# Jittor/PointCloudLib

Measured on AMD Instinct MI355X. Metric: point-clouds/sec fwd+bwd, PointNet++ SSG B=32 N=1024, higher is better.
Workload: dtype f32; 1 GPU; PointNet++ SSG cls train step (fwd+bwd+SGD), B=32/GPU, N=1024 xyz+normal, gauss_ball clouds (BASELINE configs[1]); global_batch=32, n_points=1024, parallelism=dp1, launch=eager, grad_overlap=False, cpu_affinity=numa node 1 (gpu0), 128 cpus, world_size=1, sync_bn=False, entry_points=per-stack (pcl_mlp_stack_*_f32)

## Files before the change

include/pcl_hip.h:

```cpp
#ifndef PCL_HIP_H
#define PCL_HIP_H

#include <stddef.h>
#include <stdint.h>

#ifdef __cplusplus
extern "C" {
#endif

#define PCL_OK 0
#define PCL_EINVAL (-1)
#define PCL_EHIP (-2)
#define PCL_ENOSUP (-3)
#define PCL_EWS (-4)

int pcl_version(void);
void pcl_time_tagged_launch(void* start_event, void* stop_event, const char* tag);
void pcl_time_next_launch(void* start_event, void* stop_event);
const char* pcl_last_launch_kernel(void);
const char* pcl_last_error(void);

int pcl_optimal_block(int batch_size);

void pcl_set_fps_tuning(int threads_per_cloud, int issue_priority);
// ... 48 lines not shown
                         int S, int D, float* out, void* stream);
int pcl_three_interp_bwd_f32(const float* gout, const int32_t* idx3, const float* w3, int B, int N,
                             int S, int D, float* gpoints2, void* stream);

int pcl_density_f32(const float* xyz, int B, int N, float bandwidth, float* density_out, void* stream);

int pcl_group_linear_stat_rows(int B, int m);
int pcl_group_linear_f32(const float* xyz, const float* new_xyz, const float* Uf, const float* Wx, const float* feat_small,
                         const float* Wf_small, int CF, int ldw, const int32_t* idx, const int32_t* cnt, const int32_t* group_off,
                         int B, int N, int m, int ns, int C1, float* Y, int32_t* row_meta, int32_t* row_src,
                         float* row_loc , float* row_feat ,
                         double* stats_ws, void* stream);
int pcl_group_linear_bwd_f32(const float* row_loc, const float* row_feat, int CF, const float* dU, const float* Y,
                             const float* a, const float* k1, const float* k2, const float* mu, const int32_t* row_src,
                             const int32_t* n_rows_dev , int B, int N, int C1, float* dUf,
                             float* dWx_part, float* dWf_part, float* dW0, int ldw, int off, void* stream);
int pcl_group_rows_transpose_supported(int N, int m, int ns);
int pcl_group_rows_transpose_i32(const int32_t* row_src, const int32_t* group_off, int B, int N, int m, int ns, int32_t* in_off,
                                 int32_t* in_rows, void* stream);
int pcl_group_linear_bwd_gather_supported(int C1);
void pcl_set_pointconv_paths(int bwd_w_rows);
void pcl_set_scatter_form(int gather);
int pcl_group_linear_bwd_gather_f32(const float* row_loc, const float* dU, const float* Y, const float* a, const float* k1,
                                    const float* k2, const float* mu, const int32_t* in_off, const int32_t* in_rows, int B, int N,
                                    int C1, float* dUf, float* dWx_part, float* dW0, int ldw, void* stream);
int pcl_group_linear_bwd_regen_supported(int C1, int CF);
int pcl_group_linear_bwd_regen_f32(const float* row_loc, const float* row_feat, const float* Wx, const float* Wf_small, int CF, int ldw,
                                   const float* dU, const float* a, const float* k1, const float* k2, const float* mu,
                                   const int32_t* n_rows_dev , int C1, float* dWx_part, float* dWf_part, float* dW0,
                                   int ld0, int off, void* stream);
int pcl_group_linear_bwd_gather_regen_f32(const float* row_loc, const float* dU, const float* Uf, const float* Wx, int ldw, const float* a,
                                          const float* k1, const float* k2, const float* mu, const int32_t* in_off, const int32_t* in_rows,
                                          int B, int N, int C1, float* dUf, float* dWx_part, float* dW0, int ld0, void* stream);

int pcl_head_layer_fwd_f32(const float* X, const float* W, const float* bias, const float* gamma, const float* beta,
                           float* running_mean, float* running_var, int R, int K, int N, int bn_mode, float eps, float momentum,
                           float slope, float* Ypre, float* OUT, float* mean_out, float* invstd_out, void* workspace,
                           size_t workspace_bytes, void* stream);
size_t pcl_head_layer_fwd_workspace_bytes(int R, int K, int N);
int pcl_head_layer_bwd_f32(const float* X, const float* W, const float* dOUT, const float* OUT, const float* Ypre,
                           const float* gamma, const float* mean, const float* invstd, int R, int K, int N, int bn_mode,
                           float slope, float* dY_ws, float* dW, float* dbias, float* dgamma, float* dbeta, float* dX,
                           void* stream);

#define PCL_HEAD_MAX_LAYERS 4
typedef struct pcl_head_layer_t {
    const float* W;
    const float* bias;
    const float* gamma;
    const float* beta;
    float* running_mean;
    float* running_var;
    float* dW;
    float* dbias;
    float* dgamma;
    float* dbeta;
    int32_t K, N, bn_mode;
    float eps, momentum, slope, drop_p;
    int32_t pad_;
} pcl_head_layer_t;
typedef struct pcl_fc_head_t {
    int32_t struct_bytes;
    int32_t n_layers;
    int32_t R;
    int32_t pad_;
    uint64_t seed;
// ... 44 lines not shown
                       const float* in_shift, float in_slope, int P, int Cin, int Cout, float* Y,
                       double* stats_ws, void* stream);
int pcl_linear_fwd_gmax_f32(const float* X, const float* W, const float* bias, const float* in_scale,
                            const float* in_shift, float in_slope, int P, int Cin, int Cout, int ns, float* Y,
                            double* stats_ws, float* gmax, float* gmin, int32_t* gamax, int32_t* gamin, void* stream);
int pcl_group_minmax_finalize_f32(const float* gmax, const float* gmin, const int32_t* gamax, const int32_t* gamin,
                                  const float* scale, const float* shift, float slope, int G, int C, float* out,
                                  int32_t* arg, float* ymax, void* stream);
int pcl_group_minmax_finalize2_f32(const float* gmax, const float* gmin, const int32_t* gamax, const int32_t* gamin,
                                   const float* scale, const float* shift, float slope, int G, int C, float* out,
                                   int32_t* arg, float* ymax, float* out2, int out2_ld, void* stream);
int pcl_group_minmax_finalize_t_f32(const float* gmax, const float* gmin, const int32_t* gamax, const int32_t* gamin,
                                    const float* scale, const float* shift, float slope, int B, int N, int C, float* out,
                                    int32_t* arg, float* ymax, float* out2, int out2_ld, float* out_t, void* stream);
int pcl_bn_finalize_f32(const double* stats_ws, int stat_rows, const float* gamma, const float* beta, int P,
                        int C, float eps, float momentum, float* scale, float* shift, float* mean_out,
                        float* invstd_out, float* running_mean, float* running_var, void* stream);
int pcl_bn_act_max_mean_f32(const float* Y, const float* scale, const float* shift, float slope, int G, int ns, int C, int ldo,
                            float* out_max, float* out_mean, int32_t* arg, void* stream);
int pcl_bn_act_max_mean_bwd_f32(const float* gmax, const float* gmean, int ldg, const int32_t* arg, const float* Y, const float* scale,
                                const float* shift, float slope, int G, int ns, int C, float* du, double* stats_ws,
                                int* stat_rows_out, void* stream);
int pcl_bn_act_max_f32(const float* Y, const float* scale, const float* shift, float slope, int G, int ns,
                       int C, float* out, int32_t* arg, float* ymax, void* stream);
int pcl_bn_act_f32(const float* Y, const float* scale, const float* shift, float slope, int P, int C,
                   float* out, void* stream);
int pcl_bn_act_bwd_f32(const float* gz, const float* Y, const float* scale, const float* shift, float slope,
                       int P, int C, float* du, double* stats_ws, int* stat_rows_out, void* stream);
int pcl_bn_rows_stats_f32(const float* x, const float* g, int P, int C, double* stats_ws, int* stat_rows_out, void* stream);
int pcl_bn_rows_bwd_apply_f32(const float* g, const float* x, const float* a, const float* k1, const float* k2, const float* mean,
                              int P, int C, float* dx, void* stream);
int pcl_maxgrad_prep_f32(const float* gout, const float* out, const float* ymax, float slope, int G, int C,
                         float* gz, double* stats_ws, int* stat_rows_out, void* stream);
int pcl_bn_bwd_consts_f32(const double* stats_ws, int stat_rows, const float* gamma, const float* mean,
                          const float* invstd, int P, int C, float* dgamma, float* dbeta, float* a_out,
                          float* k1, float* k2, float* dbias_zero, void* stream);
int pcl_linear_bwd_dx_f32(const float* dU, const float* Y, const float* a, const float* k1, const float* k2, const float* mu,
                          const int32_t* arg, const float* gz, int ns, const float* W, int P, int Cout,
                          int Cin, const float* Yprev, const float* prev_scale, const float* prev_shift,
                          float prev_slope, float* dUprev, double* stats_ws, void* stream);
void pcl_set_fb_max_blocks(int n);
void pcl_set_fb_two_images(int on);
int pcl_get_fb_two_images(void);
int pcl_sgd_momentum_f32(const uint64_t* params, const uint64_t* grads, const uint64_t* bufs, const int64_t* numel, int n_tensors, double lr,
                         double momentum, double weight_decay, double dampening, void* stream);
void pcl_set_kernel_paths(int fwd_resident, int narrow_stacks, int fused_backward);
void pcl_set_stack_overlap(int side_dw, int max_rows);
int pcl_get_stack_overlap(void);
int pcl_bn_bwd_dy_supported(int P, int C);
int pcl_bn_bwd_dy_f32(const double* stats_ws, int stat_rows, const float* gamma, const float* mean, const float* invstd, int P_bn, int C,
                      float* dgamma, float* dbeta, float* a_out, float* k1, float* k2, float* dbias_zero, const float* dU, const float* Y,
                      const int32_t* arg, const float* gz, int ns, int P, float* dy, void* stream);
size_t pcl_linear_bwd_dw_plain_workspace_bytes(int P, int Cout, int Cin);
int pcl_linear_bwd_dw_plain_f32(const float* dy, const float* Xprev, const float* prev_scale, const float* prev_shift, float prev_slope, int P,
                                int Cout, int Cin, float* dW, void* workspace, size_t workspace_bytes, int dw_ld, void* stream);
int pcl_mlp_fewrow_layer(int P, int Cout, int Cin, int first_layer);
void pcl_set_fewrow_backward(int on);
int pcl_get_fewrow_backward(void);
void pcl_set_dw_tuning(int gx);
int pcl_linear_bwd_pair_supported(int P, int Cout, int Cin, int first_col);
int pcl_linear_bwd_pair_f32(const float* dU, const float* Y, const float* a, const float* k1, const float* k2, const float* mean,
                            const int32_t* arg, const float* gz, int ns, const float* W, const float* Xprev,
                            const float* prev_scale, const float* prev_shift, float prev_slope, int masked, int P, int Cout, int Cin,
                            float* dUprev, double* stats_ws, int first_col, void* workspace, size_t workspace_bytes, void* stream);
int pcl_linear_bwd_pair_finish_f32(const void* workspace, size_t workspace_bytes, int P, int Cout, int Cin, float* dW, int dw_ld,
                                   const double* stats_ws, int stat_rows, const float* gamma_prev, const float* mean_prev,
                                   const float* invstd_prev, int P_bn, float* dgamma_prev, float* dbeta_prev,
                                   float* a_prev, float* k1_prev, float* k2_prev, float* dbias_zero_prev, void* stream);
void pcl_set_bwd_pair(int on);
int pcl_get_bwd_pair(void);
void pcl_set_matrix_form(int form);
int pcl_get_matrix_form(void);
int pcl_linear_bwd_fused_supported(int Cout, int Cin);
int pcl_linear_bwd_fused_stat_rows(int P, int Cin);
size_t pcl_linear_bwd_fused_workspace_bytes(int P, int Cout, int Cin);
int pcl_linear_bwd_fused_rows_f32(const float* dU, const float* Y, const float* a, const float* k1, const float* k2, const float* mu,
                                  const int32_t* arg, const float* gz, int ns, const float* W, int P, int Cout, int Cin,
                                  const float* Yprev, const float* prev_scale, const float* prev_shift, float prev_slope,
                                  float* dUprev, double* stats_ws, void* workspace, size_t workspace_bytes,
                                  const int32_t* row_meta, const int32_t* n_rows_dev, void* stream);
int pcl_linear_bwd_fused_finish_f32(const void* workspace, size_t workspace_bytes, int P, int Cout, int Cin, float* dW,
                                    const double* stats_ws, const float* gamma_prev, const float* mean_prev,
                                    const float* invstd_prev, int P_bn, float* dgamma_prev, float* dbeta_prev, float* a_prev,
                                    float* k1_prev, float* k2_prev, float* dbias_zero_prev, void* stream);
size_t pcl_linear_bwd_dw_workspace_bytes(int P, int Cout, int Cin);
int pcl_linear_bwd_dw_f32(const float* dU, const float* Y, const float* a, const float* k1, const float* k2, const float* mu,
                          const int32_t* arg, const float* gz, int ns, const float* Xprev,
                          const float* prev_scale, const float* prev_shift, float prev_slope, int P, int Cout,
                          int Cin, float* dW, void* workspace, size_t workspace_bytes, void* stream);

#define PCL_STACK_MAX_LAYERS 8
typedef struct pcl_stack_layer_t {
    const float* W;
    const float* bias;
    const float* gamma;
    const float* beta;
    float* running_mean;
    float* running_var;
    float* dW;
    float* dbias;
    float* dgamma;
// ... 176 lines not shown
```

pointcloudlib_amd/csrc/common.h:

```cpp
#pragma once
#include <hip/hip_runtime.h>
#include <hip/hip_ext.h>
#include <stdint.h>
#include <stdio.h>
#include <stdarg.h>
#include <stdlib.h>
#include "../../include/pcl_hip.h"

namespace pcl {

void set_error(const char* fmt, ...);

inline int fail(int code, const char* fmt, ...) {
    char buf[256];
    va_list ap;
    va_start(ap, fmt);
    vsnprintf(buf, sizeof buf, fmt, ap);
    va_end(ap);
    set_error("%s", buf);
    return code;
}

inline int check_launch(const char* what) {
    hipError_t e = hipGetLastError();
// ... 60 lines not shown
}

#define PCL_WAVE 64

__device__ __forceinline__ float sq_dist3(float ax, float ay, float az, float bx, float by, float bz) {
    const float dx = __fsub_rn(ax, bx), dy = __fsub_rn(ay, by), dz = __fsub_rn(az, bz);
    return __fadd_rn(__fadd_rn(__fmul_rn(dx, dx), __fmul_rn(dy, dy)), __fmul_rn(dz, dz));
}

template <int CTRL>
__device__ __forceinline__ unsigned dpp_u32(unsigned v, unsigned old) {
    return (unsigned)__builtin_amdgcn_update_dpp((int)old, (int)v, CTRL, 0xf, 0xf, false);
}

__device__ __forceinline__ unsigned wave_max_u32(unsigned v) {
    v = max(v, dpp_u32<0xB1>(v, v));
    v = max(v, dpp_u32<0x4E>(v, v));
    v = max(v, dpp_u32<0x141>(v, v));
    v = max(v, dpp_u32<0x140>(v, v));
    const unsigned a = __builtin_amdgcn_readlane(v, 0), b = __builtin_amdgcn_readlane(v, 16);
    const unsigned c = __builtin_amdgcn_readlane(v, 32), d = __builtin_amdgcn_readlane(v, 48);
    return max(max(a, b), max(c, d));
}
__device__ __forceinline__ unsigned wave_min_u32(unsigned v) {
    v = min(v, dpp_u32<0xB1>(v, v));
    v = min(v, dpp_u32<0x4E>(v, v));
    v = min(v, dpp_u32<0x141>(v, v));
    v = min(v, dpp_u32<0x140>(v, v));
    const unsigned a = __builtin_amdgcn_readlane(v, 0), b = __builtin_amdgcn_readlane(v, 16);
    const unsigned c = __builtin_amdgcn_readlane(v, 32), d = __builtin_amdgcn_readlane(v, 48);
    return min(min(a, b), min(c, d));
}

__device__ __forceinline__ int lane_id() { return (int)__builtin_amdgcn_mbcnt_hi(~0u, __builtin_amdgcn_mbcnt_lo(~0u, 0u)); }

__device__ __forceinline__ int mbcnt(unsigned long long mask) {
    return (int)__builtin_amdgcn_mbcnt_hi((unsigned)(mask >> 32), __builtin_amdgcn_mbcnt_lo((unsigned)mask, 0u));
}

}
```

pointcloudlib_amd/csrc/compact.hip:

```cpp
#include "common.h"

namespace pcl {

struct GoffMulti { const int32_t* cnt[4]; int32_t* goff[4]; };
__device__ __forceinline__ void group_offsets_body(const int32_t* __restrict__ cnt, int G, int32_t* __restrict__ goff);
__global__ __launch_bounds__(1024) void group_offsets_kernel(const int32_t* __restrict__ cnt, int G, int32_t* __restrict__ goff) {
    group_offsets_body(cnt, G, goff);
}
__global__ __launch_bounds__(1024) void group_offsets_multi_kernel(const GoffMulti a, int G) {
    group_offsets_body(a.cnt[blockIdx.x], G, a.goff[blockIdx.x]);
}
__device__ __forceinline__ void group_offsets_body(const int32_t* __restrict__ cnt, int G, int32_t* __restrict__ goff) {
    __shared__ int part[1024];
    const int t = threadIdx.x;
    const int per = (G + 1023) / 1024;
    const int lo = min(t * per, G), hi = min(lo + per, G);
    int s = 0;
    for (int g = lo; g < hi; ++g) s += max(cnt[g], 1);
    part[t] = s;
    __syncthreads();
    for (int off = 1; off < 1024; off <<= 1) {
        const int v = t >= off ? part[t - off] : 0;
        __syncthreads();
        part[t] += v;
        __syncthreads();
    }
    int run = part[t] - s;
    for (int g = lo; g < hi; ++g) { goff[g] = run; run += max(cnt[g], 1); }
    if (t == 1023) goff[G] = part[1023];
}

__global__ __launch_bounds__(256) void group_compact_kernel(const float* __restrict__ xyz, const float* __restrict__ new_xyz,
                                                            const float* __restrict__ feat, const int32_t* __restrict__ idx,
                                                            const int32_t* __restrict__ cnt, const int32_t* __restrict__ goff,
                                                            int G, int N, int m, int ns, int C, int use_xyz, int S,
                                                            float* __restrict__ rows, int2* __restrict__ rmeta,
                                                            int32_t* __restrict__ rsrc) {
    const int g = blockIdx.x, wave = threadIdx.x >> 6, lane = threadIdx.x & 63;
    const int D = (use_xyz ? 3 : 0) + C, off3 = use_xyz ? 3 : 0;
    const int c = max(cnt[g], 1), base = goff[g];
    const int b = g / m;
    const int32_t* I = idx + (size_t)g * ns;
    const int chunk = (ns + 3) >> 2;
    const int s_lo = wave * chunk, s_hi = min(s_lo + chunk, c);
    if (s_lo >= s_hi) return;
    float* o = rows + (size_t)base * S;
    const float* fb = feat ? feat + (size_t)b * N * C : nullptr;
    if (C >= 32) {
        float q[3] = {0.f, 0.f, 0.f};
        if (use_xyz && lane < 3) q[0] = new_xyz[(size_t)g * 3 + lane];
        for (int s = s_lo; s < s_hi; s += 4) {
            int k[4];
#pragma unroll
            for (int j = 0; j < 4; ++j) k[j] = I[min(s + j, s_hi - 1)];
            for (int c0 = 0; c0 < C; c0 += 128) {
                float v[4][2];
#pragma unroll
                for (int j = 0; j < 4; ++j)
#pragma unroll
                    for (int h = 0; h < 2; ++h) {
                        const int ch = min(c0 + h * 64 + lane, C - 1);
                        v[j][h] = fb[(size_t)k[j] * C + ch];
// ... 698 lines not shown
    __syncthreads();
    int run = inc - s;
    for (int w = 0; w < wave; ++w) run += wtot[w];
    for (int i = i0; i < i1; ++i) {
        const int t = off[i];
        off[i] = run;
        int pos = run;
        for (int w = 0; w < RT_W; ++w) { const int c = cnt[w * N + i]; cnt[w * N + i] = pos; pos += c; }
        run += t;
    }
    if (tid == 0) off[N] = re - rb;
    __syncthreads();
    for (int g = g0; g < g1; ++g) {
        const int q0 = group_off[g_first + g], q1 = group_off[g_first + g + 1];
        for (int r = q0 + lane; r < q1; r += 64) lst[atomicAdd(&mycnt[rsrc[r] - pbase], 1)] = r;
        __builtin_amdgcn_fence(__ATOMIC_SEQ_CST, "wavefront");
        __builtin_amdgcn_wave_barrier();
    }
    __syncthreads();
    for (int pl = tid; pl < N; pl += RT_T) in_off[pbase + pl] = rb + off[pl];
    if (b == B - 1 && tid == 0) in_off[pbase + N] = re;
    for (int i = tid; i < re - rb; i += RT_T) in_rows[rb + i] = lst[i];
}

__global__ __launch_bounds__(256) void group_linear_dw_kernel(const float* __restrict__ px, const float* __restrict__ pf, int rows,
                                                              int C1, int CF, int off, int ld, float* __restrict__ dW0) {
    const int nx = px ? C1 * 3 : 0, nf = pf ? C1 * CF : 0;
    const int e = blockIdx.x * 4 + (threadIdx.x >> 6), lane = threadIdx.x & 63;
    if (e >= nx + nf) return;
    const bool isx = e < nx;
    const float* src = isx ? px + e : pf + (e - nx);
    const int n = isx ? nx : nf;
    float s = 0.f;
    for (int r = lane; r < rows; r += 64) s += src[(size_t)r * n];
#pragma unroll
    for (int o = 32; o > 0; o >>= 1) s += __shfl_xor(s, o);
    if (lane == 0) {
        if (isx) dW0[(size_t)(e / 3) * ld + e % 3] = s;
        else dW0[(size_t)((e - nx) / CF) * ld + off + (e - nx) % CF] = s;
    }
}

}
using namespace pcl;

extern "C" int pcl_group_offsets_i32(const int32_t* cnt, int G, int32_t* group_off, void* stream) {
    PCL_REQUIRE(cnt && group_off && G >= 1, "pcl_group_offsets_i32: bad arguments");
    hipLaunchKernelGGL(group_offsets_kernel, dim3(1), dim3(1024), 0, as_stream(stream), cnt, G, group_off);
    return check_launch("pcl_group_offsets_i32");
}

extern "C" int pcl_group_offsets_multi_i32(int n, const int32_t* const* cnt, int G, int32_t* const* group_off, void* stream) {
    PCL_REQUIRE(cnt && group_off && G >= 1 && n >= 1 && n <= 4, "pcl_group_offsets_multi_i32: bad arguments (n = %d: 1..4)", n);
    GoffMulti a = {};
    for (int i = 0; i < n; ++i) {
        PCL_REQUIRE(cnt[i] && group_off[i], "pcl_group_offsets_multi_i32: null array %d", i);
        a.cnt[i] = cnt[i]; a.goff[i] = group_off[i];
    }
    hipLaunchKernelGGL(group_offsets_multi_kernel, dim3(n), dim3(1024), 0, as_stream(stream), a, G);
    return check_launch("pcl_group_offsets_multi_i32");
}

extern "C" int pcl_group_compact_f32(const float* xyz, const float* new_xyz, const float* feat, const int32_t* idx,
                                     const int32_t* cnt, const int32_t* group_off, int B, int N, int m, int ns, int C,
                                     int use_xyz, int row_stride, float* rows, int32_t* row_meta, int32_t* row_src,
                                     void* stream) {
    PCL_REQUIRE(idx && cnt && rows && row_meta && row_src && group_off, "pcl_group_compact_f32: null pointer");
// ... 106 lines not shown
    return group_linear_bwd_impl(row_loc, row_feat, CF, dU, Y, a, k1, k2, mu, row_src, n_rows_dev, B, N, C1, dUf, dWx_part, dWf_part, dW0, ldw,
                                 off, stream, false);
}
int pcl::group_linear_bwd_impl(const float* row_loc, const float* row_feat, int CF, const float* dU, const float* Y, const float* a,
                               const float* k1, const float* k2, const float* mu, const int32_t* row_src, const int32_t* n_rows_dev, int B,
                               int N, int C1, float* dUf, float* dWx_part, float* dWf_part, float* dW0, int ldw, int off, void* stream,
                               bool duf_is_zero) {
    PCL_REQUIRE(row_loc && dU && Y && a && k1 && k2 && mu && row_src && n_rows_dev, "pcl_group_linear_bwd_f32: null pointer");
    PCL_REQUIRE(dUf || dWx_part || dWf_part, "pcl_group_linear_bwd_f32: nothing to compute");
    PCL_REQUIRE(!dWf_part || (row_feat && CF >= 1 && CF <= GL_CF), "pcl_group_linear_bwd_f32: dWf needs row_feat, CF=%d", CF);
    PCL_REQUIRE(B >= 1 && N >= 1 && C1 >= 1 && C1 <= 64 * GL_MAXH, "pcl_group_linear_bwd_f32: bad sizes");
    PCL_REQUIRE(!dW0 || ((dWx_part || dWf_part) && ldw >= (dWx_part ? 3 : 0) && off >= 0 && ldw >= off + (dWf_part ? CF : 0)),
                "pcl_group_linear_bwd_f32: dW0 needs the partial buffers and ldw=%d >= off=%d + CF", ldw, off);
    hipStream_t st = as_stream(stream);
    if (dUf && !duf_is_zero) {
        hipError_t e = hipMemsetAsync(dUf, 0, sizeof(float) * (size_t)B * N * C1, st);
        if (e != hipSuccess) return fail(PCL_EHIP, "pcl_group_linear_bwd_f32: memset: %s", hipGetErrorString(e));
    }
    const float4* rl = reinterpret_cast<const float4*>(row_loc);
    const float4* rf = reinterpret_cast<const float4*>(row_feat);
    const dim3 grid(GL_BLOCKS), block(256);
    if (!dUf && al16(Y, dU) && (C1 == 64 || C1 == 128 || C1 == 256)) {
        if (C1 == 64) hipLaunchKernelGGL(group_linear_bwd_v4_kernel<16>, grid, block, 0, st, rl, rf, CF, dU, Y, a, k1, k2, mu, row_src, n_rows_dev, dUf, dWx_part, dWf_part);
        else if (C1 == 128) hipLaunchKernelGGL(group_linear_bwd_v4_kernel<32>, grid, block, 0, st, rl, rf, CF, dU, Y, a, k1, k2, mu, row_src, n_rows_dev, dUf, dWx_part, dWf_part);
        else hipLaunchKernelGGL(group_linear_bwd_v4_kernel<64>, grid, block, 0, st, rl, rf, CF, dU, Y, a, k1, k2, mu, row_src, n_rows_dev, dUf, dWx_part, dWf_part);
    } else if (C1 <= 64) hipLaunchKernelGGL(group_linear_bwd_kernel<1>, grid, block, 0, st, rl, rf, CF, dU, Y, a, k1, k2, mu, row_src, n_rows_dev, C1, dUf, dWx_part, dWf_part);
    else if (C1 <= 128) hipLaunchKernelGGL(group_linear_bwd_kernel<2>, grid, block, 0, st, rl, rf, CF, dU, Y, a, k1, k2, mu, row_src, n_rows_dev, C1, dUf, dWx_part, dWf_part);
    else hipLaunchKernelGGL(group_linear_bwd_kernel<4>, grid, block, 0, st, rl, rf, CF, dU, Y, a, k1, k2, mu, row_src, n_rows_dev, C1, dUf, dWx_part, dWf_part);
    int rc = check_launch("pcl_group_linear_bwd_f32");
    if (rc || !dW0) return rc;
    const int n = (dWx_part ? C1 * 3 : 0) + (dWf_part ? C1 * CF : 0);
    hipLaunchKernelGGL(group_linear_dw_kernel, dim3((n + 3) / 4), block, 0, st, dWx_part, dWf_part, GL_BLOCKS, C1, CF, off, ldw, dW0);
    return check_launch("pcl_group_linear_bwd_f32(dW)");
}

extern "C" int pcl_group_rows_transpose_supported(int N, int m, int ns) {
    return N >= 1 && m >= 1 && ns >= 1 && ((size_t)(RT_W + 1) * N + 1 + (size_t)m * ns) * 4 <= 150 * 1024;
}
extern "C" int pcl_group_rows_transpose_i32(const int32_t* row_src, const int32_t* group_off, int B, int N, int m, int ns, int32_t* in_off,
                                            int32_t* in_rows, void* stream) {
    PCL_REQUIRE(row_src && group_off && in_off && in_rows && B >= 1 && m >= 1 && ns >= 1, "pcl_group_rows_transpose_i32: bad arguments");
    PCL_REQUIRE(pcl_group_rows_transpose_supported(N, m, ns), "pcl_group_rows_transpose_i32: N=%d m=%d ns=%d beyond the LDS-resident form", N, m, ns);
    const size_t lds = ((size_t)(RT_W + 1) * N + 1 + (size_t)m * ns) * 4;
    auto kern = rows_transpose_kernel;
    if (int rc = lds_opt_in(kern, lds, "pcl_group_rows_transpose_i32")) return rc;
    hipLaunchKernelGGL(kern, dim3(B), dim3(RT_T), lds, as_stream(stream), row_src, group_off, m, N, B, in_off, in_rows);
    return check_launch("pcl_group_rows_transpose_i32");
}
extern "C" int pcl_group_linear_bwd_gather_supported(int C1) { return g_lab.scatter_gather && (C1 == 64 || C1 == 128 || C1 == 256); }
extern "C" int pcl_group_linear_bwd_gather_f32(const float* row_loc, const float* dU, const float* Y, const float* a, const float* k1,
                                               const float* k2, const float* mu, const int32_t* in_off, const int32_t* in_rows, int B, int N,
                                               int C1, float* dUf, float* dWx_part, float* dW0, int ldw, void* stream) {
    PCL_REQUIRE(row_loc && dU && Y && a && k1 && k2 && mu && in_off && in_rows && dUf, "pcl_group_linear_bwd_gather_f32: null pointer");
    PCL_REQUIRE(B >= 1 && N >= 1 && pcl_group_linear_bwd_gather_supported(C1), "pcl_group_linear_bwd_gather_f32: bad sizes (C1 = %d: 64, 128 or 256)", C1);
    PCL_REQUIRE(al16(dU, Y, dUf), "pcl_group_linear_bwd_gather_f32: 16-byte aligned rows");
    PCL_REQUIRE(!dW0 || (dWx_part && ldw >= 3), "pcl_group_linear_bwd_gather_f32: dW0 needs dWx_part and ldw >= 3");
    hipStream_t st = as_stream(stream);
    const float4* rl = reinterpret_cast<const float4*>(row_loc);
    const dim3 grid(GL_BLOCKS), block(256);
    const int P = B * N;
    if (C1 == 64) hipLaunchKernelGGL(group_linear_bwd_gather_kernel<16>, grid, block, 0, st, rl, dU, Y, a, k1, k2, mu, in_off, in_rows, P, dUf, dWx_part);
    else if (C1 == 128) hipLaunchKernelGGL(group_linear_bwd_gather_kernel<32>, grid, block, 0, st, rl, dU, Y, a, k1, k2, mu, in_off, in_rows, P, dUf, dWx_part);
    else hipLaunchKernelGGL(group_linear_bwd_gather_kernel<64>, grid, block, 0, st, rl, dU, Y, a, k1, k2, mu, in_off, in_rows, P, dUf, dWx_part);
    int rc = check_launch("pcl_group_linear_bwd_gather_f32");
    if (rc || !dW0) return rc;
    hipLaunchKernelGGL(group_linear_dw_kernel, dim3((C1 * 3 + 3) / 4), block, 0, st, dWx_part, (const float*)nullptr, GL_BLOCKS, C1, 0, 0, ldw, dW0);
// ... 55 lines not shown
```

pointcloudlib_amd/csrc/mlp.hip:

```cpp
#include <cstdlib>
#include "common.h"
#if defined(__HIP_DEVICE_COMPILE__) && !defined(__gfx950__)
#error "mlp.hip is written for gfx950 (MI355X) only: its buffer addressing relies on the range check covering the scalar offset (tools/ubench/bufcheck.hip)"
#endif

#ifndef PCL_EXP
#define PCL_EXP 0
#endif

namespace pcl {

typedef float f32x16 __attribute__((ext_vector_type(16)));

constexpr int BK = 32, LDS_LD = BK + 4;
constexpr int MLP_T = 256;
constexpr int STAT_ROWS = 1024;

enum AMode { A_PLAIN = 0, A_BNACT = 1, A_DY = 2, A_DY_SPARSE = 3 };
enum EMode { E_STORE_STATS = 0, E_MASK_STORE_STATS = 1, E_STORE = 2 };

struct LinArgs {
    const float* A;
    const float* A2;
    int ldb;
// ... 2403 lines not shown
        return;
    }
    if ((int)blockIdx.x >= nred) { bn_bwd_consts_block(q, blockIdx.x - nred, red); return; }
    float* redf = reinterpret_cast<float*>(red);
    const int el = threadIdx.x & 31, ry = threadIdx.x >> 5;
    const size_t e = (size_t)blockIdx.x * 32 + el;
    float acc = 0.f;
    if (e < n) {
#pragma unroll 8
        for (int r = ry; r < rows; r += 8) acc += part[(size_t)r * n + e];
    }
    redf[ry * 33 + el] = acc;
    __syncthreads();
    if (ry == 0 && e < n) {
        float t = 0.f;
#pragma unroll
        for (int j = 0; j < 8; ++j) t += redf[j * 33 + el];
        out[ldo == 0 || ldo == ncols ? e : (e / ncols) * ldo + e % ncols] = t;
    }
}

__global__ __launch_bounds__(256) void bn_act_max_kernel(const float* __restrict__ Y, const float* __restrict__ scale,
                                                         const float* __restrict__ shift, float slope, int G, int ns,
                                                         int C, float* __restrict__ out, int32_t* __restrict__ arg,
                                                         float* __restrict__ ymax) {
    const size_t total = (size_t)G * C;
    for (size_t e = (size_t)blockIdx.x * 256 + threadIdx.x; e < total; e += (size_t)gridDim.x * 256) {
        const size_t g = e / C;
        const int c = (int)(e - g * C);
        const float a = scale[c], b = shift[c];
        const float* y = Y + g * ns * C + c;
        float best = -INFINITY, by = 0.f;
        int bi = 0;
        for (int s = 0; s < ns; ++s) {
            const float yy = y[(size_t)s * C];
            const float z = lrelu(fmaf(a, yy, b), slope);
            if (z > best) { best = z; bi = s; by = yy; }
        }
        out[e] = best;
        if (arg) arg[e] = bi;
        if (ymax) ymax[e] = by;
    }
}

template <int SL>
__global__ __launch_bounds__(64 * SL) void bn_act_max_sliced_kernel(const float* __restrict__ Y, const float* __restrict__ scale,
                                                                    const float* __restrict__ shift, float slope, int ns, int C,
                                                                    float* __restrict__ out, int32_t* __restrict__ arg,
                                                                    float* __restrict__ ymax) {
    __shared__ float sz[SL][64], sy[SL][64];
    __shared__ int ss[SL][64];
    const int cl = threadIdx.x & 63, sl = threadIdx.x >> 6;
    const int c = blockIdx.x * 64 + cl, g = blockIdx.y;
    float best = -INFINITY, by = 0.f;
    int bi = 0;
    if (c < C) {
        const float a = scale[c], b = shift[c];
        const float* y = Y + (size_t)g * ns * C + c;
        for (int s = sl; s < ns; s += SL) {
            const float yy = y[(size_t)s * C];
            const float z = lrelu(fmaf(a, yy, b), slope);
            if (z > best) { best = z; bi = s; by = yy; }
        }
    }
    sz[sl][cl] = best; sy[sl][cl] = by; ss[sl][cl] = bi;
    __syncthreads();
    if (sl != 0 || c >= C) return;
#pragma unroll
    for (int j = 1; j < SL; ++j) {
        const float z = sz[j][cl];
        const int s = ss[j][cl];
        if (z > best || (z == best && s < bi)) { best = z; bi = s; by = sy[j][cl]; }
    }
    const size_t e = (size_t)g * C + c;
    out[e] = best;
    if (arg) arg[e] = bi;
    if (ymax) ymax[e] = by;
}

template <int SL>
__global__ __launch_bounds__(64 * SL) void bn_act_maxmean_sliced_kernel(const float* __restrict__ Y, const float* __restrict__ scale,
                                                                        const float* __restrict__ shift, float slope, int ns, int C, int ldo,
                                                                        float* __restrict__ out_max, float* __restrict__ out_mean,
                                                                        int32_t* __restrict__ arg) {
    __shared__ float sz[SL][64];
    __shared__ int ss[SL][64];
    __shared__ double sm[SL][64];
    const int cl = threadIdx.x & 63, sl = threadIdx.x >> 6;
    const int c = blockIdx.x * 64 + cl, g = blockIdx.y;
    float best = -INFINITY;
    int bi = 0;
    double sum = 0.0;
    if (c < C) {
        const float a = scale[c], b = shift[c];
        const float* y = Y + (size_t)g * ns * C + c;
        for (int s = sl; s < ns; s += SL) {
            const float z = lrelu(fmaf(a, y[(size_t)s * C], b), slope);
            if (z > best) { best = z; bi = s; }
            sum += (double)z;
        }
    }
    sz[sl][cl] = best; ss[sl][cl] = bi; sm[sl][cl] = sum;
    __syncthreads();
    if (sl != 0 || c >= C) return;
#pragma unroll
    for (int j = 1; j < SL; ++j) {
        const float z = sz[j][cl];
        const int s = ss[j][cl];
        if (z > best || (z == best && s < bi)) { best = z; bi = s; }
        sum += sm[j][cl];
    }
    out_max[(size_t)g * ldo + c] = best;
    out_mean[(size_t)g * ldo + c] = (float)(sum / ns);
    arg[(size_t)g * C + c] = bi;
}

__global__ __launch_bounds__(256) void group_minmax_finalize_kernel(const float* __restrict__ gmax, const float* __restrict__ gmin,
                                                                    const int32_t* __restrict__ gamax, const int32_t* __restrict__ gamin,
                                                                    const float* __restrict__ scale, const float* __restrict__ shift,
                                                                    float slope, int C, size_t total, float* __restrict__ out,
                                                                    int32_t* __restrict__ arg, float* __restrict__ ymax,
                                                                    float* __restrict__ out2 = nullptr, int ld2 = 0) {
    for (size_t e = (size_t)blockIdx.x * 256 + threadIdx.x; e < total; e += (size_t)gridDim.x * 256) {
        const int c = (int)(e % C);
        const float a = scale[c];
        const bool up = a >= 0.f;
        const float y = up ? gmax[e] : gmin[e];
        const float o = lrelu(fmaf(a, y, shift[c]), slope);
        out[e] = o;
        if (out2) out2[(e / C) * (size_t)ld2 + c] = o;
        arg[e] = up ? gamax[e] : gamin[e];
        ymax[e] = y;
    }
}

__device__ __forceinline__ void fold_row_lanes(double s1, double s2, int c, int rsub, int RS, int CW, int C, double* red,
                                               double* __restrict__ dst) {
    if (RS > 1) {
        red[(size_t)rsub * CW + (threadIdx.x % CW)] = s1;
        red[(size_t)(RS + rsub) * CW + (threadIdx.x % CW)] = s2;
        __syncthreads();
        if (rsub == 0) {
            for (int j = 1; j < RS; ++j) { s1 += red[(size_t)j * CW + threadIdx.x]; s2 += red[(size_t)(RS + j) * CW + threadIdx.x]; }
        }
    }
    if (rsub == 0 && c < C) { dst[c] = s1; dst[C + c] = s2; }
}

struct PrepAux { float4* zero; size_t n_zero4; float* ones; int n_one, n_one0; };
__global__ __launch_bounds__(256) void maxgrad_prep_kernel(const float* __restrict__ gout, const float* __restrict__ out,
                                                           const float* __restrict__ ymax, float slope, int G, int C, int CW, int ldg,
                                                           float* __restrict__ gz, double* __restrict__ stats, const PrepAux aux) {
    __shared__ double red[2 * 256];
    if (aux.zero || aux.ones) {
        const size_t nb = (size_t)gridDim.x * gridDim.y, b = (size_t)blockIdx.y * gridDim.x + blockIdx.x;
        for (size_t e = b * 256 + threadIdx.x; e < aux.n_zero4; e += nb * 256) aux.zero[e] = make_float4(0.f, 0.f, 0.f, 0.f);
        if (b == 0 && aux.ones)
            for (int e = threadIdx.x; e < aux.n_one + aux.n_one0; e += 256) aux.ones[e] = e < aux.n_one ? 1.f : 0.f;
    }
    const int RS = 256 / CW, rsub = threadIdx.x / CW;
    const int c = blockIdx.x * CW + threadIdx.x % CW;
    double s1 = 0.0, s2 = 0.0;
    if (c < C)
        for (int g = blockIdx.y * RS + rsub; g < G; g += gridDim.y * RS) {
            const size_t e = (size_t)g * C + c;
            const float v = gout[(size_t)g * ldg + c] * (out[e] > 0.f ? 1.f : slope);
            gz[e] = v;
            s1 += v; s2 += (double)v * ymax[e];
        }
    fold_row_lanes(s1, s2, c, rsub, RS, CW, C, red, stats + (size_t)blockIdx.y * 2 * C);
}

__global__ __launch_bounds__(256) void bn_act_kernel(const float* __restrict__ Y, const float* __restrict__ scale,
                                                     const float* __restrict__ shift, float slope, int C, size_t total,
                                                     float* __restrict__ out) {
    for (size_t e = (size_t)blockIdx.x * 256 + threadIdx.x; e < total; e += (size_t)gridDim.x * 256) {
        const int c = (int)(e % C);
        out[e] = lrelu(fmaf(scale[c], Y[e], shift[c]), slope);
    }
}

__global__ __launch_bounds__(256) void bn_act_bwd_kernel(const float* __restrict__ gz, const float* __restrict__ Y,
                                                         const float* __restrict__ scale, const float* __restrict__ shift,
                                                         float slope, int P, int C, int CW, float* __restrict__ du,
                                                         double* __restrict__ stats) {
    __shared__ double red[2 * 256];
    const int RS = 256 / CW, rsub = threadIdx.x / CW;
    const int c = blockIdx.x * CW + threadIdx.x % CW;
    double s1 = 0.0, s2 = 0.0;
    if (c < C) {
        const float a = scale[c], b = shift[c];
        for (int r = blockIdx.y * RS + rsub; r < P; r += gridDim.y * RS) {
            const size_t e = (size_t)r * C + c;
            const float y = Y[e];
            const float v = gz[e] * (fmaf(a, y, b) > 0.f ? 1.f : slope);
            du[e] = v;
            s1 += v; s2 += (double)v * y;
        }
    }
    fold_row_lanes(s1, s2, c, rsub, RS, CW, C, red, stats + (size_t)blockIdx.y * 2 * C);
}

// ... 382 lines not shown
        if (dU) { if (vec_dw) launch_dw_t<A_DY, true>(d, dim3(n_dw), tm, tn, st); else launch_dw_t<A_DY, false>(d, dim3(n_dw), tm, tn, st); }
        else { if (vec_dw) launch_dw_t<A_DY_SPARSE, true>(d, dim3(n_dw), tm, tn, st); else launch_dw_t<A_DY_SPARSE, false>(d, dim3(n_dw), tm, tn, st); }
        if (const int rc = check_launch("pcl_linear_bwd_pair_f32(dw)")) return rc;
        return launch_linear(a, st);
    }
    const bool vec = vec_dw;
    const dim3 grid(n_dw + gxl * n_tiles), blk(MLP_T);
#define PCL_PAIR(AMv, EMv, VECv) PCL_LAUNCH_TIMED((linear_bwd_pair_kernel<AMv, EMv, VECv>), grid, blk, st, d, a, n_dw)
    if (dU) {
        if (masked) { if (vec) PCL_PAIR(A_DY, E_MASK_STORE_STATS, true); else PCL_PAIR(A_DY, E_MASK_STORE_STATS, false); }
        else { if (vec) PCL_PAIR(A_DY, E_STORE, true); else PCL_PAIR(A_DY, E_STORE, false); }
    } else {
        if (masked) { if (vec) PCL_PAIR(A_DY_SPARSE, E_MASK_STORE_STATS, true); else PCL_PAIR(A_DY_SPARSE, E_MASK_STORE_STATS, false); }
        else { if (vec) PCL_PAIR(A_DY_SPARSE, E_STORE, true); else PCL_PAIR(A_DY_SPARSE, E_STORE, false); }
    }
#undef PCL_PAIR
    return check_launch("pcl_linear_bwd_pair_f32");
}

namespace pcl {
int pair_finish_impl(const void* workspace, size_t workspace_bytes, int P, int Cout, int Cin, float* dW, int dw_ld,
                     const double* stats_ws, int stat_rows, const float* gamma_prev, const float* mean_prev,
                     const float* invstd_prev, int P_bn, float* dgamma_prev, float* dbeta_prev,
                     float* a_prev, float* k1_prev, float* k2_prev, float* dbias_zero_prev, void* stream,
                     const float* xpart, int xrows, int xC1, int xld, float* xdW0);
}
extern "C" int pcl_linear_bwd_pair_finish_f32(const void* workspace, size_t workspace_bytes, int P, int Cout, int Cin, float* dW, int dw_ld,
                                              const double* stats_ws, int stat_rows, const float* gamma_prev, const float* mean_prev,
                                              const float* invstd_prev, int P_bn, float* dgamma_prev, float* dbeta_prev,
                                              float* a_prev, float* k1_prev, float* k2_prev, float* dbias_zero_prev, void* stream) {
    return pair_finish_impl(workspace, workspace_bytes, P, Cout, Cin, dW, dw_ld, stats_ws, stat_rows, gamma_prev, mean_prev, invstd_prev, P_bn, dgamma_prev,
                            dbeta_prev, a_prev, k1_prev, k2_prev, dbias_zero_prev, stream, nullptr, 0, 0, 0, nullptr);
}
int pcl::pair_finish_impl(const void* workspace, size_t workspace_bytes, int P, int Cout, int Cin, float* dW, int dw_ld,
                          const double* stats_ws, int stat_rows, const float* gamma_prev, const float* mean_prev,
                          const float* invstd_prev, int P_bn, float* dgamma_prev, float* dbeta_prev,
                          float* a_prev, float* k1_prev, float* k2_prev, float* dbias_zero_prev, void* stream,
                          const float* xpart, int xrows, int xC1, int xld, float* xdW0) {
    PCL_REQUIRE(workspace && dW && P >= 1 && Cout >= 1 && Cin >= 1 && (dw_ld == 0 || dw_ld >= Cin), "pcl_linear_bwd_pair_finish_f32: bad arguments");
    const size_t need = pcl_linear_bwd_dw_workspace_bytes(P, Cout, Cin);
    if (workspace_bytes < need) return fail(PCL_EWS, "pcl_linear_bwd_pair_finish_f32: workspace %zu < %zu", workspace_bytes, need);
    int gx, ti, tj, tm, tn;
    dw_grid(P, Cout, Cin, gx, ti, tj, tm, tn);
    BnConstsArgs q = {};
    int extra = 0;
    if (stats_ws) {
        PCL_REQUIRE(mean_prev && invstd_prev && a_prev && k1_prev && k2_prev && P_bn >= 1 && stat_rows >= 1, "pcl_linear_bwd_pair_finish_f32: null pointer");
        q = BnConstsArgs{stats_ws, stat_rows, gamma_prev, mean_prev, invstd_prev, P_bn, Cin, dgamma_prev, dbeta_prev, a_prev, k1_prev, k2_prev, dbias_zero_prev};
        extra = (Cin + 3) / 4;
    }
    const size_t n = (size_t)Cout * Cin;
    const int nred = (int)((n + 31) / 32);
    FinishXJob xj = {nullptr, 0, 0, 0, nullptr, 0};
    int xblocks = 0;
    if (xpart && xdW0) { xj = FinishXJob{xpart, xrows, xC1, xld, xdW0, nred + extra}; xblocks = (xC1 * 3 + 3) / 4; }
    hipLaunchKernelGGL(fused_finish_kernel, dim3(nred + extra + xblocks), dim3(256), 0, as_stream(stream), static_cast<const float*>(workspace), gx, n, Cin, dW, nred, q,
                       dw_ld, xj);
    return check_launch("pcl_linear_bwd_pair_finish_f32");
}

extern "C" int pcl_bn_bwd_dy_supported(int P, int C) { return P >= 1 && C >= 32 && C % 32 == 0; }

extern "C" int pcl_bn_bwd_dy_f32(const double* stats_ws, int stat_rows, const float* gamma, const float* mean, const float* invstd, int P_bn, int C,
                                 float* dgamma, float* dbeta, float* a_out, float* k1, float* k2, float* dbias_zero, const float* dU, const float* Y,
                                 const int32_t* arg, const float* gz, int ns, int P, float* dy, void* stream) {
    PCL_REQUIRE(stats_ws && mean && invstd && a_out && k1 && k2 && Y && dy, "pcl_bn_bwd_dy_f32: null pointer");
// ... 187 lines not shown
                                       float* out_max, float* out_mean, int32_t* arg, void* stream) {
    PCL_REQUIRE(Y && scale && shift && out_max && out_mean && arg, "pcl_bn_act_max_mean_f32: null pointer");
    PCL_REQUIRE(G >= 1 && G <= 65535 && ns >= 1 && C >= 1 && ldo >= C, "pcl_bn_act_max_mean_f32: bad sizes G=%d ns=%d C=%d ldo=%d", G, ns, C, ldo);
    const dim3 grid((C + 63) / 64, G);
    if (ns >= 256) hipLaunchKernelGGL(bn_act_maxmean_sliced_kernel<16>, grid, dim3(1024), 0, as_stream(stream), Y, scale, shift, slope, ns, C, ldo, out_max, out_mean, arg);
    else hipLaunchKernelGGL(bn_act_maxmean_sliced_kernel<4>, grid, dim3(256), 0, as_stream(stream), Y, scale, shift, slope, ns, C, ldo, out_max, out_mean, arg);
    return check_launch("pcl_bn_act_max_mean_f32");
}

extern "C" int pcl_bn_act_max_mean_bwd_f32(const float* gmax, const float* gmean, int ldg, const int32_t* arg, const float* Y, const float* scale,
                                           const float* shift, float slope, int G, int ns, int C, float* du, double* stats_ws,
                                           int* stat_rows_out, void* stream) {
    PCL_REQUIRE(gmax && gmean && arg && Y && scale && shift && du && stats_ws && stat_rows_out, "pcl_bn_act_max_mean_bwd_f32: null pointer");
    PCL_REQUIRE(G >= 1 && ns >= 1 && C >= 1 && ldg >= C && (size_t)G * ns < 0x7fffffffull, "pcl_bn_act_max_mean_bwd_f32: bad sizes G=%d ns=%d C=%d ldg=%d", G, ns, C, ldg);
    const int P = G * ns;
    int CW = 256;
    while (CW / 2 >= C && CW > 1) CW >>= 1;
    const int RS = 256 / CW;
    const int rows = (P + RS - 1) / RS < STAT_ROWS ? (P + RS - 1) / RS : STAT_ROWS;
    *stat_rows_out = rows;
    hipLaunchKernelGGL(bn_act_maxmean_bwd_kernel, dim3((C + CW - 1) / CW, rows), dim3(256), 0, as_stream(stream), gmax, gmean, ldg, arg, Y, scale, shift,
                       slope, G, ns, C, CW, du, stats_ws);
    return check_launch("pcl_bn_act_max_mean_bwd_f32");
}

namespace pcl {
int maxgrad_prep_impl(const float* gout, const float* out, const float* ymax, float slope, int G, int C, float* gz, double* stats_ws,
                      int* stat_rows_out, void* stream, float* zero, size_t n_zero, float* ones, int n_one, int n_one0, int ldg);
}
extern "C" int pcl_maxgrad_prep_f32(const float* gout, const float* out, const float* ymax, float slope, int G, int C,
                                    float* gz, double* stats_ws, int* stat_rows_out, void* stream) {
    return maxgrad_prep_impl(gout, out, ymax, slope, G, C, gz, stats_ws, stat_rows_out, stream, nullptr, 0, nullptr, 0, 0, C);
}
int pcl::maxgrad_prep_impl(const float* gout, const float* out, const float* ymax, float slope, int G, int C, float* gz, double* stats_ws,
                           int* stat_rows_out, void* stream, float* zero, size_t n_zero, float* ones, int n_one, int n_one0, int ldg) {
    PCL_REQUIRE(gout && out && ymax && gz && stats_ws && stat_rows_out, "pcl_maxgrad_prep_f32: null pointer");
    PCL_REQUIRE(ldg >= C, "pcl_maxgrad_prep_f32: gout row stride %d below the width %d", ldg, C);
    PCL_REQUIRE(!zero || (al16(zero) && n_zero % 4 == 0), "pcl_maxgrad_prep_f32: the zero-fill region must be 16-byte aligned and a multiple of 4 floats");
    const PrepAux aux = {reinterpret_cast<float4*>(zero), n_zero / 4, ones, n_one, n_one0};
    PCL_REQUIRE(G >= 1 && C >= 1, "pcl_maxgrad_prep_f32: bad sizes");
    int CW = 256;
    while (CW / 2 >= C && CW > 1) CW >>= 1;
    const int RS = 256 / CW;
    int rows = (G + RS - 1) / RS < 512 ? (G + RS - 1) / RS : 512;
    *stat_rows_out = rows;
    hipLaunchKernelGGL(maxgrad_prep_kernel, dim3((C + CW - 1) / CW, rows), dim3(256), 0, as_stream(stream), gout, out, ymax,
                       slope, G, C, CW, ldg, gz, stats_ws, aux);
    return check_launch("pcl_maxgrad_prep_f32");
}

extern "C" int pcl_bn_act_f32(const float* Y, const float* scale, const float* shift, float slope, int P, int C,
                              float* out, void* stream) {
    PCL_REQUIRE(Y && scale && shift && out && P >= 1 && C >= 1, "pcl_bn_act_f32: bad arguments");
    const size_t total = (size_t)P * C;
    int blocks = (int)((total + 255) / 256);
    if (blocks > 8192) blocks = 8192;
    hipLaunchKernelGGL(bn_act_kernel, dim3(blocks), dim3(256), 0, as_stream(stream), Y, scale, shift, slope, C, total, out);
    return check_launch("pcl_bn_act_f32");
}

extern "C" int pcl_bn_act_bwd_f32(const float* gz, const float* Y, const float* scale, const float* shift, float slope,
                                  int P, int C, float* du, double* stats_ws, int* stat_rows_out, void* stream) {
    PCL_REQUIRE(gz && Y && scale && shift && du && stats_ws && stat_rows_out && P >= 1 && C >= 1, "pcl_bn_act_bwd_f32: bad arguments");
    int CW = 256;
    while (CW / 2 >= C && CW > 1) CW >>= 1;
    const int RS = 256 / CW;
// ... 31 lines not shown
```

Baseline: 18410 point-clouds/s.

## Keep multiple strided row loads in flight across reduction kernels

```diff
diff --git a/include/pcl_hip.h b/include/pcl_hip.h
--- a/include/pcl_hip.h
+++ b/include/pcl_hip.h
@@ -104,6 +104,8 @@
 int pcl_group_linear_bwd_gather_regen_f32(const float* row_loc, const float* dU, const float* Uf, const float* Wx, int ldw, const float* a,
                                           const float* k1, const float* k2, const float* mu, const int32_t* in_off, const int32_t* in_rows,
                                           int B, int N, int C1, float* dUf, float* dWx_part, float* dW0, int ld0, void* stream);
+int pcl_group_linear_dw_sum_f32(const float* dWx_part, const float* dWf_part, int rows, int C1, int CF, int off, int ld, float* dW0,
+                                void* stream);
 
 int pcl_head_layer_fwd_f32(const float* X, const float* W, const float* bias, const float* gamma, const float* beta,
                            float* running_mean, float* running_var, int R, int K, int N, int bn_mode, float eps, float momentum,
@@ -214,6 +216,8 @@
                               int P, int C, float* dx, void* stream);
 int pcl_maxgrad_prep_f32(const float* gout, const float* out, const float* ymax, float slope, int G, int C,
                          float* gz, double* stats_ws, int* stat_rows_out, void* stream);
+int pcl_maxgrad_prep_ld_f32(const float* gout, int ldg, const float* out, const float* ymax, float slope, int G, int C,
+                            float* gz, double* stats_ws, int* stat_rows_out, void* stream);
 int pcl_bn_bwd_consts_f32(const double* stats_ws, int stat_rows, const float* gamma, const float* mean,
                           const float* invstd, int P, int C, float* dgamma, float* dbeta, float* a_out,
                           float* k1, float* k2, float* dbias_zero, void* stream);
@@ -249,6 +253,11 @@
                                    const double* stats_ws, int stat_rows, const float* gamma_prev, const float* mean_prev,
                                    const float* invstd_prev, int P_bn, float* dgamma_prev, float* dbeta_prev,
                                    float* a_prev, float* k1_prev, float* k2_prev, float* dbias_zero_prev, void* stream);
+int pcl_linear_bwd_pair_finish_xyz_f32(const void* workspace, size_t workspace_bytes, int P, int Cout, int Cin, float* dW, int dw_ld,
+                                       const double* stats_ws, int stat_rows, const float* gamma_prev, const float* mean_prev,
+                                       const float* invstd_prev, int P_bn, float* dgamma_prev, float* dbeta_prev,
+                                       float* a_prev, float* k1_prev, float* k2_prev, float* dbias_zero_prev,
+                                       const float* xpart, int xrows, int xC1, int xld, float* xdW0, void* stream);
 void pcl_set_bwd_pair(int on);
 int pcl_get_bwd_pair(void);
 void pcl_set_matrix_form(int form);
diff --git a/pointcloudlib_amd/csrc/common.h b/pointcloudlib_amd/csrc/common.h
--- a/pointcloudlib_amd/csrc/common.h
+++ b/pointcloudlib_amd/csrc/common.h
@@ -116,6 +116,21 @@
     return min(min(a, b), min(c, d));
 }
 
+template <int U, class L, class F>
+__device__ __forceinline__ void rows_in_flight(int r, int step, int n, L&& load, F&& use) {
+    for (; r + (U - 1) * step < n; r += U * step) {
+        decltype(load(r)) v[U];
+#pragma unroll
+        for (int u = 0; u < U; ++u) v[u] = load(r + u * step);
+#pragma unroll
+        for (int u = 0; u < U; ++u) use(r + u * step, v[u]);
+    }
+    if constexpr (U > 1) rows_in_flight<U / 2>(r, step, n, load, use);
+}
+template <int U, class T, class F>
+__device__ __forceinline__ void rows_in_flight(const T* __restrict__ x, size_t ld, int r, int step, int n, F&& use) {
+    rows_in_flight<U>(r, step, n, [&](int q) { return x[(size_t)q * ld]; }, use);
+}
 __device__ __forceinline__ int lane_id() { return (int)__builtin_amdgcn_mbcnt_hi(~0u, __builtin_amdgcn_mbcnt_lo(~0u, 0u)); }
 
 __device__ __forceinline__ int mbcnt(unsigned long long mask) {
diff --git a/pointcloudlib_amd/csrc/compact.hip b/pointcloudlib_amd/csrc/compact.hip
--- a/pointcloudlib_amd/csrc/compact.hip
+++ b/pointcloudlib_amd/csrc/compact.hip
@@ -11,23 +11,29 @@
     group_offsets_body(a.cnt[blockIdx.x], G, a.goff[blockIdx.x]);
 }
 __device__ __forceinline__ void group_offsets_body(const int32_t* __restrict__ cnt, int G, int32_t* __restrict__ goff) {
-    __shared__ int part[1024];
-    const int t = threadIdx.x;
-    const int per = (G + 1023) / 1024;
-    const int lo = min(t * per, G), hi = min(lo + per, G);
+    __shared__ int tot[16];
+    constexpr int U = 8;
+    const int lane = threadIdx.x & 63, w = threadIdx.x >> 6;
+    const int per = ((G + 15) / 16 + 63) / 64 * 64;
+    const int lo = min(w * per, G), hi = min(lo + per, G);
     int s = 0;
-    for (int g = lo; g < hi; ++g) s += max(cnt[g], 1);
-    part[t] = s;
+    rows_in_flight<U>(cnt, 1, lo + lane, 64, hi, [&](int, int v) { s += max(v, 1); });
+#pragma unroll
+    for (int o = 32; o > 0; o >>= 1) s += __shfl_xor(s, o);
+    if (lane == 0) tot[w] = s;
     __syncthreads();
-    for (int off = 1; off < 1024; off <<= 1) {
-        const int v = t >= off ? part[t - off] : 0;
-        __syncthreads();
-        part[t] += v;
-        __syncthreads();
-    }
-    int run = part[t] - s;
-    for (int g = lo; g < hi; ++g) { goff[g] = run; run += max(cnt[g], 1); }
-    if (t == 1023) goff[G] = part[1023];
+    int run = 0, all = 0;
+#pragma unroll
+    for (int j = 0; j < 16; ++j) { const int t = tot[j]; run += j < w ? t : 0; all += t; }
+    rows_in_flight<U>(lo, 64, hi, [&](int g0) { return max(cnt[min(g0 + lane, hi - 1)], 1); },
+                      [&](int g0, int v) {
+                          int inc = v;
+#pragma unroll
+                          for (int o = 1; o < 64; o <<= 1) { const int t = __shfl_up(inc, o); if (lane >= o) inc += t; }
+                          if (g0 + lane < hi) goff[g0 + lane] = run + inc - v;
+                          run += __shfl(inc, 63);
+                      });
+    if (threadIdx.x == 0) goff[G] = all;
 }
 
 __global__ __launch_bounds__(256) void group_compact_kernel(const float* __restrict__ xyz, const float* __restrict__ new_xyz,
@@ -792,7 +798,7 @@
     const float* src = isx ? px + e : pf + (e - nx);
     const int n = isx ? nx : nf;
     float s = 0.f;
-    for (int r = lane; r < rows; r += 64) s += src[(size_t)r * n];
+    rows_in_flight<8>(src, n, lane, 64, rows, [&](int, float v) { s += v; });
 #pragma unroll
     for (int o = 32; o > 0; o >>= 1) s += __shfl_xor(s, o);
     if (lane == 0) {
@@ -965,6 +971,16 @@
     const int n = (dWx_part ? C1 * 3 : 0) + (dWf_part ? C1 * CF : 0);
     hipLaunchKernelGGL(group_linear_dw_kernel, dim3((n + 3) / 4), block, 0, st, dWx_part, dWf_part, GL_BLOCKS, C1, CF, off, ldw, dW0);
     return check_launch("pcl_group_linear_bwd_f32(dW)");
+}
+
+extern "C" int pcl_group_linear_dw_sum_f32(const float* dWx_part, const float* dWf_part, int rows, int C1, int CF, int off, int ld, float* dW0,
+                                           void* stream) {
+    PCL_REQUIRE((dWx_part || dWf_part) && dW0 && rows >= 1 && C1 >= 1, "pcl_group_linear_dw_sum_f32: bad arguments");
+    PCL_REQUIRE(!dWf_part || CF >= 1, "pcl_group_linear_dw_sum_f32: dWf_part needs CF >= 1");
+    PCL_REQUIRE(ld >= (dWx_part ? 3 : 0) && off >= 0 && ld >= off + (dWf_part ? CF : 0), "pcl_group_linear_dw_sum_f32: ld=%d below off=%d + CF", ld, off);
+    const int n = (dWx_part ? C1 * 3 : 0) + (dWf_part ? C1 * CF : 0);
+    hipLaunchKernelGGL(group_linear_dw_kernel, dim3((n + 3) / 4), dim3(256), 0, as_stream(stream), dWx_part, dWf_part, rows, C1, CF, off, ld, dW0);
+    return check_launch("pcl_group_linear_dw_sum_f32");
 }
 
 extern "C" int pcl_group_rows_transpose_supported(int N, int m, int ns) {
diff --git a/pointcloudlib_amd/csrc/mlp.hip b/pointcloudlib_amd/csrc/mlp.hip
--- a/pointcloudlib_amd/csrc/mlp.hip
+++ b/pointcloudlib_amd/csrc/mlp.hip
@@ -2459,11 +2459,10 @@
         const float* y = Y + g * ns * C + c;
         float best = -INFINITY, by = 0.f;
         int bi = 0;
-        for (int s = 0; s < ns; ++s) {
-            const float yy = y[(size_t)s * C];
+        rows_in_flight<8>(y, C, 0, 1, ns, [&](int s, float yy) {
             const float z = lrelu(fmaf(a, yy, b), slope);
             if (z > best) { best = z; bi = s; by = yy; }
-        }
+        });
         out[e] = best;
         if (arg) arg[e] = bi;
         if (ymax) ymax[e] = by;
@@ -2484,11 +2483,10 @@
     if (c < C) {
         const float a = scale[c], b = shift[c];
         const float* y = Y + (size_t)g * ns * C + c;
-        for (int s = sl; s < ns; s += SL) {
-            const float yy = y[(size_t)s * C];
+        rows_in_flight<8>(y, C, sl, SL, ns, [&](int s, float yy) {
             const float z = lrelu(fmaf(a, yy, b), slope);
             if (z > best) { best = z; bi = s; by = yy; }
-        }
+        });
     }
     sz[sl][cl] = best; sy[sl][cl] = by; ss[sl][cl] = bi;
     __syncthreads();
@@ -2521,11 +2519,11 @@
     if (c < C) {
         const float a = scale[c], b = shift[c];
         const float* y = Y + (size_t)g * ns * C + c;
-        for (int s = sl; s < ns; s += SL) {
-            const float z = lrelu(fmaf(a, y[(size_t)s * C], b), slope);
+        rows_in_flight<8>(y, C, sl, SL, ns, [&](int s, float yy) {
+            const float z = lrelu(fmaf(a, yy, b), slope);
             if (z > best) { best = z; bi = s; }
             sum += (double)z;
-        }
+        });
     }
     sz[sl][cl] = best; ss[sl][cl] = bi; sm[sl][cl] = sum;
     __syncthreads();
@@ -2588,13 +2586,16 @@
     const int RS = 256 / CW, rsub = threadIdx.x / CW;
     const int c = blockIdx.x * CW + threadIdx.x % CW;
     double s1 = 0.0, s2 = 0.0;
-    if (c < C)
-        for (int g = blockIdx.y * RS + rsub; g < G; g += gridDim.y * RS) {
-            const size_t e = (size_t)g * C + c;
-            const float v = gout[(size_t)g * ldg + c] * (out[e] > 0.f ? 1.f : slope);
-            gz[e] = v;
-            s1 += v; s2 += (double)v * ymax[e];
-        }
+    if (c < C) {
+        struct Row { float g, o, y; };
+        rows_in_flight<8>(blockIdx.y * RS + rsub, gridDim.y * RS, G,
+                          [&](int g) { const size_t e = (size_t)g * C + c; return Row{gout[(size_t)g * ldg + c], out[e], ymax[e]}; },
+                          [&](int g, const Row& r) {
+                              const float v = r.g * (r.o > 0.f ? 1.f : slope);
+                              gz[(size_t)g * C + c] = v;
+                              s1 += v; s2 += (double)v * r.y;
+                          });
+    }
     fold_row_lanes(s1, s2, c, rsub, RS, CW, C, red, stats + (size_t)blockIdx.y * 2 * C);
 }
 
@@ -3043,6 +3044,15 @@
     return pair_finish_impl(workspace, workspace_bytes, P, Cout, Cin, dW, dw_ld, stats_ws, stat_rows, gamma_prev, mean_prev, invstd_prev, P_bn, dgamma_prev,
                             dbeta_prev, a_prev, k1_prev, k2_prev, dbias_zero_prev, stream, nullptr, 0, 0, 0, nullptr);
 }
+extern "C" int pcl_linear_bwd_pair_finish_xyz_f32(const void* workspace, size_t workspace_bytes, int P, int Cout, int Cin, float* dW, int dw_ld,
+                                                  const double* stats_ws, int stat_rows, const float* gamma_prev, const float* mean_prev,
+                                                  const float* invstd_prev, int P_bn, float* dgamma_prev, float* dbeta_prev,
+                                                  float* a_prev, float* k1_prev, float* k2_prev, float* dbias_zero_prev,
+                                                  const float* xpart, int xrows, int xC1, int xld, float* xdW0, void* stream) {
+    PCL_REQUIRE(!xpart || (xdW0 && xrows >= 1 && xC1 >= 1 && xld >= 3), "pcl_linear_bwd_pair_finish_xyz_f32: xpart needs xdW0, xrows, xC1 >= 1 and xld >= 3");
+    return pair_finish_impl(workspace, workspace_bytes, P, Cout, Cin, dW, dw_ld, stats_ws, stat_rows, gamma_prev, mean_prev, invstd_prev, P_bn, dgamma_prev,
+                            dbeta_prev, a_prev, k1_prev, k2_prev, dbias_zero_prev, stream, xpart, xrows, xC1, xld, xdW0);
+}
 int pcl::pair_finish_impl(const void* workspace, size_t workspace_bytes, int P, int Cout, int Cin, float* dW, int dw_ld,
                           const double* stats_ws, int stat_rows, const float* gamma_prev, const float* mean_prev,
                           const float* invstd_prev, int P_bn, float* dgamma_prev, float* dbeta_prev,
@@ -3296,6 +3306,10 @@
                                     float* gz, double* stats_ws, int* stat_rows_out, void* stream) {
     return maxgrad_prep_impl(gout, out, ymax, slope, G, C, gz, stats_ws, stat_rows_out, stream, nullptr, 0, nullptr, 0, 0, C);
 }
+extern "C" int pcl_maxgrad_prep_ld_f32(const float* gout, int ldg, const float* out, const float* ymax, float slope, int G, int C,
+                                       float* gz, double* stats_ws, int* stat_rows_out, void* stream) {
+    return maxgrad_prep_impl(gout, out, ymax, slope, G, C, gz, stats_ws, stat_rows_out, stream, nullptr, 0, nullptr, 0, 0, ldg);
+}
 int pcl::maxgrad_prep_impl(const float* gout, const float* out, const float* ymax, float slope, int G, int C, float* gz, double* stats_ws,
                            int* stat_rows_out, void* stream, float* zero, size_t n_zero, float* ones, int n_one, int n_one0, int ldg) {
     PCL_REQUIRE(gout && out && ymax && gz && stats_ws && stat_rows_out, "pcl_maxgrad_prep_f32: null pointer");
```

Result: faster. 18600 point-clouds/s, median of 6 (+1.1%).
